# davidbau/rewriting

Measured on AMD Instinct MI355X. Metric: images/sec StyleGANv2-1024 fwd, higher is better.
Workload: dtype f32 (conv operands split into exact f16 pairs from 32x32 up, f32 accumulate); 1 GPU; stylegan2-1024 generator forward (FFHQ-1024 architecture); batch_per_gpu=64, mconv=seq, weights=synthetic seed 0, parallelism=seeds partitioned per rank, no collective, matrix_mode=split, direct_sums=auto

## Files before the change

rewriting_amd/csrc/rw_dconv.hip:

```cpp
#include "rw_common.h"

struct DconvProblem {
  const float* x; const unsigned char* wp; float* y;
  const float* style; const float* demod; const float* noise; const float* noise_w; const float* bias; int act;
  const float* post;
  const float* rgb_weight; const float* rgb_style; const float* rgb_bias; const float* rgb_skip; float* rgb_out;
  float rgb_scale;
  int batch, in_ch, out_ch, h, w;
  int tiles_x, tiles_y, o_tiles;
  int strided;
  float w_scale;
  float u_inv;
  const float* x_amax; float* y_amax;
};

#ifndef DC_ABL
#define DC_ABL 0
#endif
#define DC_PW 34
#ifndef DC_PROF
#define DC_PROF 0
#endif
#if DC_PROF
__device__ unsigned long long dc_prof[32];
extern "C" int rw_dconv_prof(unsigned long long* out) {
  return (int)hipMemcpyFromSymbol(out, HIP_SYMBOL(dc_prof), sizeof(unsigned long long) * 32);
}
#define DC_T() ((unsigned long long)clock64())
#endif

#ifndef DC_PRODUCTS
#define DC_PRODUCTS 3
#endif

__device__ __forceinline__ float dc_row_sum(float v) {
  v += __builtin_bit_cast(float, __builtin_amdgcn_update_dpp(0, __builtin_bit_cast(int, v), 0xB1, 0xf, 0xf, false));
  v += __builtin_bit_cast(float, __builtin_amdgcn_update_dpp(0, __builtin_bit_cast(int, v), 0x4E, 0xf, 0xf, false));
  v += __builtin_bit_cast(float, __builtin_amdgcn_update_dpp(0, __builtin_bit_cast(int, v), 0x141, 0xf, 0xf, false));
  v += __builtin_bit_cast(float, __builtin_amdgcn_update_dpp(0, __builtin_bit_cast(int, v), 0x140, 0xf, 0xf, false));
  return v;
}

template <int MODE, int WM>
__device__ __forceinline__ void dconv_body(const DconvProblem& p) {
  constexpr bool UP = MODE == 1, RGB = MODE == 2, RGBP = MODE == 3;
  static_assert(!RGB || WM == 1, "ToRGB: one wave holds all out-channels of its pixels");
  static_assert(!UP || WM == 2, "UP: the wave pairs are the two row phases");
  constexpr int WN = 4 / WM, TR = 4 * WN, PR = TR + 2;
  constexpr int NPIX = PR * DC_PW;
  constexpr int SI = (NPIX + 63) / 64;
  constexpr int BUFB = NPIX * 64;
  constexpr int VCH = 32 * WM;
  __shared__ __attribute__((aligned(16))) unsigned char Ls[2 * BUFB];
  __shared__ __attribute__((aligned(16))) float St[512];
  __shared__ float Ct[2][VCH];
  __shared__ float Cr[3][(RGB || RGBP) ? 32 * WM : 1];
  __shared__ float Red[4];

  const int tid = threadIdx.x, lane = tid & 63;
  const int wave = __builtin_amdgcn_readfirstlane(tid >> 6);
  const int wm = wave / WN, wn = wave % WN;
  const int lk = lane >> 4, lt = lane & 15;

  const int local = rw_xcd_remap(blockIdx.x, gridDim.x);
  const int ot = local % p.o_tiles;
  int pg = local / p.o_tiles;
  const int tx = pg % p.tiles_x; pg /= p.tiles_x;
  const int ty = pg % p.tiles_y;
  const int ib = pg / p.tiles_y;
  const int y0 = ty * TR, x0 = tx * 32;
  const int64_t hw = (int64_t)p.h * p.w;
  const int NC = p.in_ch >> 4, T = 9 * NC;
  const int real_ch = UP ? p.out_ch >> 2 : p.out_ch;

  float in_scale, out_scale;
  {
    float smax = p.style ? 0.f : 1.f;
    if (p.style)
      for (int i = tid; i < p.in_ch; i += 256) smax = fmaxf(smax, fabsf(p.style[(int64_t)ib * p.in_ch + i]));
    smax = rw_wave_max(smax);
    if (lane == 0) Red[wave] = smax;
    __syncthreads();
    smax = fmaxf(fmaxf(Red[0], Red[1]), fmaxf(Red[2], Red[3]));
    const float am = rw_bound_load(p.x_amax) * smax;
    int e = (int)((__float_as_uint(am) >> 23) & 0xff) - 126;
    e = e < -100 ? -100 : (e > 100 ? 100 : e);
    in_scale = __uint_as_float((unsigned)(127 + 14 - e) << 23);
    out_scale = __uint_as_float((unsigned)(127 + e - 14) << 23) * p.u_inv;
  }
  const float gain = p.act ? 1.4142135623730951f : 1.f, slope = p.act ? 0.2f : 1.f;
  for (int i = tid; i < p.in_ch; i += 256) St[i] = (p.style ? p.style[(int64_t)ib * p.in_ch + i] : 1.0f) * in_scale;
  if (tid < VCH) {
    const int o = UP ? 16 * ot + (tid & 15) : ot * VCH + tid;
    Ct[0][tid] = (p.demod ? p.demod[(int64_t)ib * real_ch + o] * p.w_scale : p.w_scale) * out_scale * gain;
    Ct[1][tid] = p.act ? p.bias[o] * gain : 0.f;
    if (RGB || RGBP) {
      const float sr = p.rgb_scale * p.rgb_style[(int64_t)ib * p.out_ch + o];
#pragma unroll
      for (int cc = 0; cc < 3; ++cc) Cr[cc][tid] = sr * p.rgb_weight[cc * p.out_ch + o];
    }
  }
  const float noise_wg = p.noise ? p.noise_w[0] * gain : 0.f;
  __syncthreads();

  const __amdgpu_buffer_rsrc_t xsrc = __builtin_amdgcn_make_buffer_rsrc(
      const_cast<float*>(p.x + (int64_t)ib * p.in_ch * hw), 0, (int)((int64_t)p.in_ch * hw * 4), 0x00020000);
  const int hw4 = (int)hw * 4;
  int xoff[SI], loff[SI];
#pragma unroll
  for (int s = 0; s < SI; ++s) {
    const int pi = 64 * s + lane;
    const int r = pi / DC_PW, cc = pi - r * DC_PW;
    const int iy = y0 - 1 + r, ix = x0 - 1 + cc;
    const bool ok = pi < NPIX && iy >= 0 && iy < p.h && ix >= 0 && ix < p.w;
    xoff[s] = ok ? (iy * p.w + ix) * 4 : 0x7fffffff;
    loff[s] = pi < NPIX ? pi * 64 + ((wave ^ rw_swz(cc)) << 4) : -1;
  }
  constexpr int SH = (SI + 1) / 2;
  float raw[SH][4];
  auto stage_load = [&](int c, auto half_tag) __attribute__((always_inline)) {
    constexpr int S0 = decltype(half_tag)::value ? SH : 0, S1 = decltype(half_tag)::value ? SI : SH;
    const int s0 = (16 * c + 4 * wave) * hw4;
#pragma unroll
    for (int s = S0; s < S1; ++s)
#pragma unroll
      for (int k = 0; k < 4; ++k)
        raw[s - S0][k] = (DC_ABL & 1) ? 1.f : __uint_as_float(__builtin_amdgcn_raw_buffer_load_b32(xsrc, xoff[s], s0 + k * hw4, 0));
  };
  auto stage_store = [&](int c, int buf, auto half_tag) __attribute__((always_inline)) {
    constexpr int S0 = decltype(half_tag)::value ? SH : 0, S1 = decltype(half_tag)::value ? SI : SH;
    const rw_f32x4 sv = *reinterpret_cast<const rw_f32x4*>(&St[16 * c + 4 * wave]);
    unsigned char* dst = Ls + buf * BUFB;
#pragma unroll
    for (int s = S0; s < S1; ++s) {
      const float (&rw)[4] = raw[s - S0];
      const float v0 = rw[0] * sv[0], v1 = rw[1] * sv[1], v2 = rw[2] * sv[2], v3 = rw[3] * sv[3];
      const rw_f16x2 h01 = __builtin_convertvector(rw_f32x2{v0, v1}, rw_f16x2);
      const rw_f16x2 h23 = __builtin_convertvector(rw_f32x2{v2, v3}, rw_f16x2);
      float r0, r1, r2, r3;
      asm("v_fma_mix_f32 %0, -%1, 1.0, %2 op_sel_hi:[1,0,0]" : "=v"(r0) : "v"(h01), "v"(v0));
      asm("v_fma_mix_f32 %0, -%1, 1.0, %2 op_sel:[1,0,0] op_sel_hi:[1,0,0]" : "=v"(r1) : "v"(h01), "v"(v1));
      asm("v_fma_mix_f32 %0, -%1, 1.0, %2 op_sel_hi:[1,0,0]" : "=v"(r2) : "v"(h23), "v"(v2));
      asm("v_fma_mix_f32 %0, -%1, 1.0, %2 op_sel:[1,0,0] op_sel_hi:[1,0,0]" : "=v"(r3) : "v"(h23), "v"(v3));
      const rw_f16x2 l01 = __builtin_convertvector(rw_f32x2{r0, r1}, rw_f16x2);
      const rw_f16x2 l23 = __builtin_convertvector(rw_f32x2{r2, r3}, rw_f16x2);
      const rw_f16x8 word = {h01[0], h01[1], h23[0], h23[1], l01[0], l01[1], l23[0], l23[1]};
      if (loff[s] >= 0) *reinterpret_cast<rw_f16x8*>(dst + loff[s]) = word;
    }
  };

  const int vb0 = ot * (2 * WM) + 2 * wm;
  const unsigned char* wbase = p.wp + (int64_t)vb0 * T * 1024 + lane * 8;
  rw_f16x8 W[3][2][2];
  rw_f32x2 Wc[3][2][2];
  auto wload = [&](int ky, int t) __attribute__((always_inline)) {
#pragma unroll
    for (int ob = 0; ob < 2; ++ob)
#pragma unroll
      for (int part = 0; part < 2; ++part) {
        if (DC_ABL & 4) Wc[ky][ob][part] = rw_f32x2{1.f, 1.f};
        else Wc[ky][ob][part] = *reinterpret_cast<const rw_f32x2*>(wbase + ((int64_t)ob * T + t) * 1024 + part * 512);
      }
  };
  auto wexpand = [&](int ky) __attribute__((always_inline)) {
#pragma unroll
    for (int ob = 0; ob < 2; ++ob) {
      W[ky][ob][0] = rw_expand(Wc[ky][ob][0]);
      if (DC_PRODUCTS == 4 || ky == 2) W[ky][ob][1] = rw_expand(Wc[ky][ob][1]);
      else if (ky == 1) W[0][ob][1] = rw_pair(Wc[0][ob][1], Wc[1][ob][1]);
    }
  };

  rw_f32x4 acc[2][8];
#pragma unroll
  for (int ob = 0; ob < 2; ++ob)
#pragma unroll
    for (int pb = 0; pb < 8; ++pb) acc[ob][pb] = rw_f32x4{0.f, 0.f, 0.f, 0.f};

  unsigned bbase[3];
#pragma unroll
  for (int kx = 0; kx < 3; ++kx) {
    const int cc = lt + kx;
    bbase[kx] = (unsigned)((4 * wn * DC_PW + cc) * 64 + ((lk ^ rw_swz(cc)) << 4));
  }
  auto bread = [&](const unsigned char* lb, int kx, int idx) __attribute__((always_inline)) {
    return *reinterpret_cast<const rw_f16x8*>(lb + bbase[kx] + ((idx >> 1) * DC_PW + 16 * (idx & 1)) * 64);
  };

  auto chunk = [&](int c, auto last_tag) __attribute__((always_inline)) {
    constexpr bool LAST = decltype(last_tag)::value != 0;
    const int buf = c & 1;
    const unsigned char* lb = Ls + buf * BUFB;
    if (!LAST) stage_load(c + 1, rw_int<0>());
    rw_f16x8 bcur = bread(lb, 0, 0);
    rw_f16x8 bprev[2] = {bcur, bcur};
#pragma unroll
    for (int kx = 0; kx < 3; ++kx) {
      const bool more = !LAST || kx < 2;
      const int tn = kx < 2 ? 9 * c + kx + 1 : 9 * (c + 1);
#pragma unroll
      for (int idx = 0; idx < 12; ++idx) {
        const int r = idx >> 1, half = idx & 1;
        if (half == 0 && r < 3) wexpand(r);
        rw_f16x8 bnext = bcur;
        if (idx + 1 < 12) bnext = bread(lb, kx, idx + 1);
        else if (kx < 2) bnext = bread(lb, kx + 1, 0);
#pragma unroll
        for (int ky = 0; ky < 3; ++ky) {
          const int pr = r - ky;
          if (pr < 0 || pr > 3) continue;
          const int pb = 2 * pr + half;
          if (DC_ABL & 2) { asm volatile("" :: "v"(bcur), "v"(W[ky][0][0]), "v"(W[ky][0][1]), "v"(W[ky][1][0]), "v"(W[ky][1][1])); continue; }
          acc[0][pb] = __builtin_amdgcn_mfma_f32_16x16x32_f16(bcur, W[ky][0][0], acc[0][pb], 0, 0, 0);
          acc[1][pb] = __builtin_amdgcn_mfma_f32_16x16x32_f16(bcur, W[ky][1][0], acc[1][pb], 0, 0, 0);
          if (DC_PRODUCTS == 4 || ky == 2) {
            acc[0][pb] = __builtin_amdgcn_mfma_f32_16x16x32_f16(bcur, W[ky][0][1], acc[0][pb], 0, 0, 0);
            acc[1][pb] = __builtin_amdgcn_mfma_f32_16x16x32_f16(bcur, W[ky][1][1], acc[1][pb], 0, 0, 0);
          }
        }
        if (DC_PRODUCTS == 3 && r >= 1 && r <= 4 && !(DC_ABL & 2)) {
          const int pb = 2 * (r - 1) + half;
          const rw_f16x8 hh = rw_pair(bprev[half], bcur);
          acc[0][pb] = __builtin_amdgcn_mfma_f32_16x16x32_f16(hh, W[0][0][1], acc[0][pb], 0, 0, 0);
          acc[1][pb] = __builtin_amdgcn_mfma_f32_16x16x32_f16(hh, W[0][1][1], acc[1][pb], 0, 0, 0);
        }
        bprev[half] = bcur;
        __builtin_amdgcn_sched_barrier(0);
        if (more && half == 1 && r >= 3) wload(r - 3, tn + 3 * (r - 3));
        bcur = bnext;
      }
      if (!LAST && kx == 0) {
        stage_store(c + 1, buf ^ 1, rw_int<0>());
        stage_load(c + 1, rw_int<1>());
      }
      __builtin_amdgcn_sched_barrier(0);
    }
    if (!LAST) {
      stage_store(c + 1, buf ^ 1, rw_int<1>());
      __syncthreads();
    }
  };

  wload(0, 0);
  wload(1, 3);
  wload(2, 6);
  stage_load(0, rw_int<0>());
  stage_store(0, 0, rw_int<0>());
  stage_load(0, rw_int<1>());
  stage_store(0, 0, rw_int<1>());
  __syncthreads();

  for (int c = 0; c + 1 < NC; ++c) chunk(c, rw_int<0>());
  chunk(NC - 1, rw_int<1>());
  if (DC_ABL & 8) { if (acc[0][0][0] != 12345.f) return; }

  float ymax = 0.f;
  if (MODE == 0 || RGBP) {
    const int oc = 16 * (2 * wm) + lt;
    const float sc[2] = {Ct[0][oc], Ct[0][oc + 16]}, bs[2] = {Ct[1][oc], Ct[1][oc + 16]};
    float* yb = p.y + ((int64_t)ib * p.out_ch + ot * VCH + oc) * hw;
    float cr[2][3] = {{0.f, 0.f, 0.f}, {0.f, 0.f, 0.f}};
    float* rb = nullptr;
    if (RGBP) {
#pragma unroll
      for (int ob = 0; ob < 2; ++ob)
#pragma unroll
        for (int cc = 0; cc < 3; ++cc) cr[ob][cc] = Cr[cc][oc + 16 * ob];
      rb = p.rgb_out + (((int64_t)(ot * WM + wm) * p.batch + ib) * 3 + (lt < 3 ? lt : 0)) * hw;
    }
#pragma unroll
    for (int pb = 0; pb < 8; ++pb) {
      const int64_t pix = (int64_t)(y0 + 4 * wn + (pb >> 1)) * p.w + x0 + 16 * (pb & 1) + 4 * lk;
      rw_f32x4 nz = {0.f, 0.f, 0.f, 0.f};
      if (p.noise) nz = *reinterpret_cast<const rw_f32x4*>(p.noise + (int64_t)ib * hw + pix) * noise_wg;
      rw_f32x4 v[2];
#pragma unroll
      for (int ob = 0; ob < 2; ++ob) {
#pragma unroll
        for (int j = 0; j < 4; ++j) {
          const float u = acc[ob][pb][j] * sc[ob] + nz[j] + bs[ob];
          v[ob][j] = fmaxf(u, u * slope);
          ymax = fmaxf(ymax, fabsf(v[ob][j]));
        }
        *reinterpret_cast<rw_f32x4*>(yb + (int64_t)(16 * ob) * hw + pix) = v[ob];
      }
      if (RGBP) {
        rw_f32x4 sum[3];
#pragma unroll
        for (int j = 0; j < 4; ++j)
#pragma unroll
          for (int cc = 0; cc < 3; ++cc) sum[cc][j] = dc_row_sum(v[0][j] * cr[0][cc] + v[1][j] * cr[1][cc]);
        if (lt < 3) *reinterpret_cast<rw_f32x4*>(rb + pix) = lt == 0 ? sum[0] : (lt == 1 ? sum[1] : sum[2]);
      }
    }
  } else if (UP) {
    const float sc = Ct[0][lt], bs = Ct[1][lt];
    const int ch = 16 * ot + lt;
    const float post = p.post ? p.post[(int64_t)ib * real_ch + ch] : 1.f;
    const int W2 = 2 * p.w;
    const int64_t hw2 = 4 * hw;
    float* yb = p.y + ((int64_t)ib * real_ch + ch) * hw2;
#pragma unroll
    for (int pb = 0; pb < 8; ++pb) {
      const int64_t pix = (int64_t)(2 * (y0 + 4 * wn + (pb >> 1)) + wm) * W2 + 2 * (x0 + 16 * (pb & 1) + 4 * lk);
      rw_f32x4 n0 = {0.f, 0.f, 0.f, 0.f}, n1 = n0;
      if (p.noise) {
        const float* np = p.noise + (int64_t)ib * hw2 + pix;
        n0 = *reinterpret_cast<const rw_f32x4*>(np) * noise_wg;
        n1 = *reinterpret_cast<const rw_f32x4*>(np + 4) * noise_wg;
      }
      rw_f32x4 q0 = {acc[0][pb][0], acc[1][pb][0], acc[0][pb][1], acc[1][pb][1]};
      rw_f32x4 q1 = {acc[0][pb][2], acc[1][pb][2], acc[0][pb][3], acc[1][pb][3]};
#pragma unroll
      for (int k = 0; k < 4; ++k) {
        const float u0 = q0[k] * sc + n0[k] + bs, u1 = q1[k] * sc + n1[k] + bs;
        q0[k] = fmaxf(u0, u0 * slope) * post; q1[k] = fmaxf(u1, u1 * slope) * post;
        ymax = fmaxf(ymax, fmaxf(fabsf(q0[k]), fabsf(q1[k])));
      }
      *reinterpret_cast<rw_f32x4*>(yb + pix) = q0;
      *reinterpret_cast<rw_f32x4*>(yb + pix + 4) = q1;
    }
  } else {
    const float sc[2] = {Ct[0][lt], Ct[0][lt + 16]}, bs[2] = {Ct[1][lt], Ct[1][lt + 16]};
    float cr[2][3];
#pragma unroll
    for (int ob = 0; ob < 2; ++ob)
#pragma unroll
      for (int cc = 0; cc < 3; ++cc) cr[ob][cc] = Cr[cc][lt + 16 * ob];
#pragma unroll
    for (int pb = 0; pb < 8; ++pb) {
      const int64_t pix = (int64_t)(y0 + 4 * wn + (pb >> 1)) * p.w + x0 + 16 * (pb & 1) + 4 * lk;
      rw_f32x4 nz = {0.f, 0.f, 0.f, 0.f};
      if (p.noise) nz = *reinterpret_cast<const rw_f32x4*>(p.noise + (int64_t)ib * hw + pix) * noise_wg;
      rw_f32x4 sum[3];
#pragma unroll
      for (int j = 0; j < 4; ++j) {
        float u0 = acc[0][pb][j] * sc[0] + nz[j] + bs[0], u1 = acc[1][pb][j] * sc[1] + nz[j] + bs[1];
        u0 = fmaxf(u0, u0 * slope); u1 = fmaxf(u1, u1 * slope);
#pragma unroll
        for (int cc = 0; cc < 3; ++cc) sum[cc][j] = dc_row_sum(u0 * cr[0][cc] + u1 * cr[1][cc]);
      }
      if (lt < 3) {
        const rw_f32x4 mine = lt == 0 ? sum[0] : (lt == 1 ? sum[1] : sum[2]);
        const int64_t off = ((int64_t)ib * 3 + lt) * hw + pix;
        rw_f32x4 o4 = mine + (p.rgb_bias ? p.rgb_bias[lt] : 0.f);
        if (p.rgb_skip) o4 += *reinterpret_cast<const rw_f32x4*>(p.rgb_skip + off);
        *reinterpret_cast<rw_f32x4*>(p.rgb_out + off) = o4;
      }
    }
  }
  if (!RGB && p.y_amax) rw_bound_store_wave(p.y_amax, rw_wave_max(ymax));
}

template <int MODE, int WM, int MW, int NL, int WC>
__device__ __forceinline__ void dconv_ws_body(const DconvProblem& p) {
  constexpr bool UP = MODE == 1, RGB = MODE == 2, RGBP = MODE == 3, PLAIN = MODE == 0 || MODE == 3;
  static_assert(!RGB || WM == 1, "ToRGB: one wave holds all out-channels of its pixels");
  static_assert(!UP || WM == 2, "UP: the wave pairs are the two row phases");
  constexpr int WN = MW / WM, WR = WN / WC, TR = 4 * WR, PR = TR + 2, TC = 32 * WC, PW = TC + 2;
  static_assert(WR * WC == WN && WR >= 1, "strips tile the workgroup's pixels");
  constexpr int QW = 4 / NL, NLL = 64 * NL;
  constexpr int NPIX = PR * PW, BUFB = NPIX * 64;
  constexpr int IPR = TC / 4 + 2, NITEM = PR * IPR, SI = (NITEM + 63) / 64;
  constexpr int VCH = 32 * WM;
  constexpr int WBUF = 2 * WM * 9 * 1024;
  __shared__ __attribute__((aligned(16))) unsigned char Ls[2 * BUFB];
  __shared__ __attribute__((aligned(16))) unsigned char Wl[2 * WBUF];
  __shared__ float Ct[2][2][VCH];
  __shared__ float Cr[2][3][VCH];
  __shared__ float Po[2][16];

  const int tid = threadIdx.x, lane = tid & 63;
  const int wave = __builtin_amdgcn_readfirstlane(tid >> 6);
  const int64_t hw = (int64_t)p.h * p.w;
  const int NC = p.in_ch >> 4, T = 9 * NC;
  const int real_ch = UP ? p.out_ch >> 2 : p.out_ch;
  const float gain = p.act ? 1.4142135623730951f : 1.f, slope = p.act ? 0.2f : 1.f;

  const int64_t total = (int64_t)p.batch * p.tiles_y * p.tiles_x * p.o_tiles;
  const int per = (int)((total + gridDim.x - 1) / gridDim.x);
  const int bx = p.strided ? rw_xcd_remap(blockIdx.x, gridDim.x) : blockIdx.x;
  const int t0 = p.strided ? 0 : bx * per;
  const int t1 = p.strided ? (int)((total - bx + gridDim.x - 1) / gridDim.x)
                           : (int)((int64_t)t0 + per < total ? t0 + per : total);
  if (t0 >= t1) {
    if (!RGB && p.y_amax) rw_bound_store_wave(p.y_amax, 0.f);
    return;
  }
  const int N = (t1 - t0) * NC;
  const int t_mul = p.strided ? gridDim.x : 1, t_add = p.strided ? bx : 0;
  auto decode = [&](int pos, int& ot, int& tx, int& ty, int& ib) __attribute__((always_inline)) {
    const int tile = pos * t_mul + t_add;
    ot = tile % p.o_tiles;
    int pg = tile / p.o_tiles;
    tx = pg % p.tiles_x; pg /= p.tiles_x;
    ty = pg % p.tiles_y;
    ib = pg / p.tiles_y;
  };
  auto lds_barrier = [&]() __attribute__((always_inline)) {
    asm volatile("" ::: "memory");
    __builtin_amdgcn_s_waitcnt(0xC07F);
    __builtin_amdgcn_s_barrier();
    asm volatile("" ::: "memory");
  };

  if (wave >= MW) {
    const int g2 = QW * (wave - MW), lid = (wave - MW) * 64 + lane;
    const float xam = rw_bound_load(p.x_amax);
    const int hw4 = (int)hw * 4;
    int loff[SI];
#pragma unroll
    for (int s = 0; s < SI; ++s) {
      const int it = 64 * s + lane;
      const int r = it / IPR, j = it - r * IPR;
      loff[s] = it < NITEM ? (r * PW + 4 * j - 3) * 64 : -1000000;
    }
    int l_tile = t0, l_c = 0, l_ib = -1, l_ot = 0, l_y0 = 0, l_x0 = 0;
    float in_scale = 1.f, out_scale = 1.f;
    int xoff[SI];
    __amdgpu_buffer_rsrc_t xsrc = __builtin_amdgcn_make_buffer_rsrc(const_cast<float*>(p.x), 0, 0, 0x00020000);
    rw_f32x4 raw[QW][SI][4];
    float psv[QW][4];
    float a_demod = 1.f, a_bias = 0.f, a_rgb = 0.f, a_post = 1.f, a_oscale = 1.f, a_iscale = 1.f;
    float a_crw[3] = {0.f, 0.f, 0.f};
    bool a_first = false;
    int a_par = 0;
    float crw[3] = {0.f, 0.f, 0.f};
    if (RGB && lid < 32) {
#pragma unroll
      for (int cc = 0; cc < 3; ++cc) crw[cc] = p.rgb_weight[cc * p.out_ch + lid] * p.rgb_scale;
    }

    float sv[QW][4];
    int l_s0 = 0;
    const unsigned char* l_wsrc = p.wp;
    auto setup = [&]() __attribute__((always_inline)) {
      if (l_tile >= t1) { l_tile = t1 - 1; l_c = NC - 1; }
      a_first = l_c == 0;
      if (l_c == 0) {
        int tx, ty, ib;
        decode(l_tile, l_ot, tx, ty, ib);
        l_y0 = ty * TR; l_x0 = tx * TC;
        if (ib != l_ib) {
          l_ib = ib;
          float smax = 0.f;
          for (int i = lane; i < p.in_ch; i += 64) smax = fmaxf(smax, fabsf(p.style[(int64_t)ib * p.in_ch + i]));
          smax = rw_wave_max(smax);
          const float am = xam * smax;
          int e = (int)((__float_as_uint(am) >> 23) & 0xff) - 126;
          e = e < -100 ? -100 : (e > 100 ? 100 : e);
          in_scale = __uint_as_float((unsigned)(127 + 14 - e) << 23);
          out_scale = __uint_as_float((unsigned)(127 + e - 14) << 23) * p.u_inv;
          xsrc = __builtin_amdgcn_make_buffer_rsrc(const_cast<float*>(p.x + (int64_t)ib * p.in_ch * hw), 0,
                                                   (int)((int64_t)p.in_ch * hw * 4), 0x00020000);
        }
#pragma unroll
        for (int s = 0; s < SI; ++s) {
          const int it = 64 * s + lane;
          const int r = it / IPR, j = it - r * IPR;
          const int iy = l_y0 - 1 + r, ix = l_x0 - 4 + 4 * j;
          const bool ok = it < NITEM && iy >= 0 && iy < p.h && ix >= 0 && ix < p.w;
          xoff[s] = ok ? (iy * p.w + ix) * 4 : 0x7ffffff0;
        }
        a_par = (l_tile - t0) & 1;
        a_oscale = out_scale;
        if (lid < VCH) {
          const int o = UP ? 16 * l_ot + (lid & 15) : l_ot * VCH + lid;
          a_demod = p.demod ? p.demod[(int64_t)l_ib * real_ch + o] : 1.f;
          a_bias = p.act ? p.bias[o] : 0.f;
          if (RGB || RGBP) a_rgb = p.rgb_style[(int64_t)l_ib * p.out_ch + o];
          if (RGBP) {
#pragma unroll
            for (int cc = 0; cc < 3; ++cc) a_crw[cc] = p.rgb_weight[cc * p.out_ch + o] * p.rgb_scale;
          }
          if (UP && lid < 16 && p.post) a_post = p.post[(int64_t)l_ib * real_ch + o];
        }
      }
#pragma unroll
      for (int q = 0; q < QW; ++q)
#pragma unroll
        for (int k = 0; k < 4; ++k) psv[q][k] = p.style[(int64_t)l_ib * p.in_ch + 16 * l_c + 4 * (g2 + q) + k];
      a_iscale = in_scale;
      l_s0 = (16 * l_c + 4 * g2) * hw4;
      l_wsrc = p.wp + ((int64_t)(l_ot * (2 * WM) + (wave - MW)) * T + 9 * l_c) * 1024;
      if (++l_c == NC) { l_c = 0; ++l_tile; }
    };
    static_assert(NL == 2 * WM && SI == 3, "wave j stages weight block j, three tap pieces per pixel piece");
    rw_f32x4 wraw[SI][3];
    auto request_s = [&](int s) __attribute__((always_inline)) {
#pragma unroll
      for (int q = 0; q < QW; ++q)
#pragma unroll
        for (int k = 0; k < 4; ++k) {
          if (DC_ABL & 1) raw[q][s][k] = rw_f32x4{1.f, 1.f, 1.f, 1.f};
          else raw[q][s][k] = __builtin_bit_cast(rw_f32x4, __builtin_amdgcn_raw_buffer_load_b128(xsrc, xoff[s], l_s0 + (4 * q + k) * hw4, 0));
        }
#pragma unroll
      for (int k = 0; k < 3; ++k) {
        if (DC_ABL & 4) wraw[s][k] = rw_f32x4{1.f, 1.f, 1.f, 1.f};
        else wraw[s][k] = *reinterpret_cast<const rw_f32x4*>(l_wsrc + (3 * s + k) * 1024 + lane * 16);
      }
    };
    auto tables = [&]() __attribute__((always_inline)) {
#pragma unroll
      for (int q = 0; q < QW; ++q)
#pragma unroll
        for (int k = 0; k < 4; ++k) sv[q][k] = psv[q][k] * a_iscale;
      if (a_first) {
        if (lid < VCH) {
          Ct[a_par][0][lid] = a_demod * p.w_scale * a_oscale * gain;
          Ct[a_par][1][lid] = a_bias * gain;
          if (RGB || RGBP) {
#pragma unroll
            for (int cc = 0; cc < 3; ++cc) Cr[a_par][cc][lid] = a_rgb * (RGBP ? a_crw[cc] : crw[cc]);
          }
          if (UP && lid < 16) Po[a_par][lid] = a_post;
        }
      }
    };
    auto deliver_s = [&](int buf, int s) __attribute__((always_inline)) {
      unsigned char* dst = Ls + buf * BUFB;
      unsigned char* wdst = Wl + buf * WBUF + (wave - MW) * 9216 + lane * 16;
#pragma unroll
      for (int k = 0; k < 3; ++k) *reinterpret_cast<rw_f32x4*>(wdst + (3 * s + k) * 1024) = wraw[s][k];
      const int it = 64 * s + lane;
      const int j = it % IPR;
#pragma unroll
      for (int q = 0; q < QW; ++q)
#pragma unroll
        for (int e = 0; e < 4; ++e) {
          const float v0 = raw[q][s][0][e] * sv[q][0], v1 = raw[q][s][1][e] * sv[q][1], v2 = raw[q][s][2][e] * sv[q][2],
                      v3 = raw[q][s][3][e] * sv[q][3];
          const rw_f16x2 h01 = __builtin_convertvector(rw_f32x2{v0, v1}, rw_f16x2);
          const rw_f16x2 h23 = __builtin_convertvector(rw_f32x2{v2, v3}, rw_f16x2);
          float r0, r1, r2, r3;
          asm("v_fma_mix_f32 %0, -%1, 1.0, %2 op_sel_hi:[1,0,0]" : "=v"(r0) : "v"(h01), "v"(v0));
          asm("v_fma_mix_f32 %0, -%1, 1.0, %2 op_sel:[1,0,0] op_sel_hi:[1,0,0]" : "=v"(r1) : "v"(h01), "v"(v1));
          asm("v_fma_mix_f32 %0, -%1, 1.0, %2 op_sel_hi:[1,0,0]" : "=v"(r2) : "v"(h23), "v"(v2));
          asm("v_fma_mix_f32 %0, -%1, 1.0, %2 op_sel:[1,0,0] op_sel_hi:[1,0,0]" : "=v"(r3) : "v"(h23), "v"(v3));
          const rw_f16x2 l01 = __builtin_convertvector(rw_f32x2{r0, r1}, rw_f16x2);
          const rw_f16x2 l23 = __builtin_convertvector(rw_f32x2{r2, r3}, rw_f16x2);
          const rw_f16x8 word = {h01[0], h01[1], h23[0], h23[1], l01[0], l01[1], l23[0], l23[1]};
          const int cc = 4 * j - 3 + e;
          if (it < NITEM && cc >= 0 && cc < PW)
            *reinterpret_cast<rw_f16x8*>(dst + loff[s] + e * 64 + (((g2 + q) ^ rw_swz(cc)) << 4)) = word;
        }
    };

    setup();
#pragma unroll
    for (int s = 0; s < SI; ++s) request_s(s);
    tables();
    __builtin_amdgcn_sched_barrier(0);
    setup();
#pragma unroll
    for (int s = 0; s < SI; ++s) { deliver_s(0, s); __builtin_amdgcn_sched_barrier(0); request_s(s); __builtin_amdgcn_sched_barrier(0); }
    lds_barrier();
#if DC_PROF
    unsigned long long pt_del = 0, pt_req = 0, pt_bar = 0, pt_all = DC_T();
#endif
    for (int n = 0; n < N; ++n) {
#if DC_PROF
      const unsigned long long ta = DC_T();
#endif
      tables();
      __builtin_amdgcn_sched_barrier(0);
      setup();
#if DC_PROF
      const unsigned long long tb = DC_T();
#endif
#pragma unroll
      for (int s = 0; s < SI; ++s) { deliver_s((n + 1) & 1, s); __builtin_amdgcn_sched_barrier(0); request_s(s); __builtin_amdgcn_sched_barrier(0); }
#if DC_PROF
      const unsigned long long tc = DC_T();
#endif
      lds_barrier();
#if DC_PROF
      const unsigned long long td = DC_T();
      pt_del += tb - ta; pt_req += tc - tb; pt_bar += td - tc;
#endif
    }
#if DC_PROF
    if (wave == MW && lane == 0 && (blockIdx.x == 0 || blockIdx.x == 100)) {
      unsigned long long* o = dc_prof + (blockIdx.x == 0 ? 0 : 16);
      o[8] = DC_T() - pt_all; o[9] = pt_del; o[10] = pt_req; o[11] = pt_bar; o[12] = N;
    }
#endif
    if (!RGB && p.y_amax) rw_bound_store_wave(p.y_amax, 0.f);
    return;
  }

  const int wm = wave / WN, wn = wave % WN, wr = wn / WC, wc = wn % WC;
  const int lk = lane >> 4, lt = lane & 15;
  unsigned bbase[3];
#pragma unroll
  for (int kx = 0; kx < 3; ++kx) {
    const int cc = lt + kx;
    bbase[kx] = (unsigned)((4 * wr * PW + 32 * wc + cc) * 64 + ((lk ^ rw_swz(cc)) << 4));
  }
  auto bread = [&](const unsigned char* lb, int kx, int idx) __attribute__((always_inline)) {
    return *reinterpret_cast<const rw_f16x8*>(lb + bbase[kx] + ((idx >> 1) * PW + 16 * (idx & 1)) * 64);
  };
  rw_f16x8 W[3][2];
  rw_f32x2 Wc[3][2];
  auto wread = [&](const unsigned char* wb, int kx, int part) __attribute__((always_inline)) {
#pragma unroll
    for (int ky = 0; ky < 3; ++ky)
#pragma unroll
      for (int ob = 0; ob < 2; ++ob) {
        if (DC_ABL & 4) Wc[ky][ob] = rw_f32x2{1.f, 1.f};
        else Wc[ky][ob] = *reinterpret_cast<const rw_f32x2*>(wb + ((2 * wm + ob) * 9 + 3 * ky + kx) * 1024 + part * 512 + lane * 8);
      }
  };
  const float noise_wg = p.noise ? p.noise_w[0] * gain : 0.f;
  rw_f32x4 nzp[PLAIN ? 8 : 1];
  rw_f32x4 acc[2][8];
#pragma unroll
  for (int ob = 0; ob < 2; ++ob)
#pragma unroll
    for (int pb = 0; pb < 8; ++pb) acc[ob][pb] = rw_f32x4{0.f, 0.f, 0.f, 0.f};
  float ymax = 0.f;
  float rgb_b[3] = {0.f, 0.f, 0.f};
  if (RGB && p.rgb_bias) { rgb_b[0] = p.rgb_bias[0]; rgb_b[1] = p.rgb_bias[1]; rgb_b[2] = p.rgb_bias[2]; }

  int tile = t0, c = 0;
  int ot, tx, ty, ib;
  decode(tile, ot, tx, ty, ib);
  lds_barrier();

#if DC_PROF
  unsigned long long pt_mm = 0, pt_bar = 0, pt_epi = 0, pt_all = DC_T();
#endif
  for (int n = 0; n < N; ++n) {
#if DC_PROF
    const unsigned long long ta = DC_T();
#endif
    const unsigned char* lb = Ls + (n & 1) * BUFB;
    const unsigned char* wb = Wl + (n & 1) * WBUF;
    if (PLAIN && c == NC - 1 && p.noise) {
      const float* np = p.noise + (int64_t)ib * hw + (int64_t)(ty * TR + 4 * wr) * p.w + tx * TC + 32 * wc + 4 * lk;
#pragma unroll
      for (int pb = 0; pb < 8; ++pb) nzp[pb] = *reinterpret_cast<const rw_f32x4*>(np + (int64_t)(pb >> 1) * p.w + 16 * (pb & 1));
    }
    rw_f16x8 bq[3];
    wread(wb, 0, 0);
    bq[0] = bread(lb, 0, 0);
    bq[1] = bread(lb, 0, 1);
    rw_f16x8 bprev[2] = {bq[0], bq[1]};
#pragma unroll
    for (int hs = 0; hs < 6; ++hs) {
      const int kx = hs >> 1, part = hs & 1;
#pragma unroll
      for (int ob = 0; ob < 2; ++ob) {
        if (DC_PRODUCTS == 4 || part == 0) {
#pragma unroll
          for (int ky = 0; ky < 3; ++ky) W[ky][ob] = rw_expand(Wc[ky][ob]);
        } else {
          W[0][ob] = rw_pair(Wc[0][ob], Wc[1][ob]);
          W[2][ob] = rw_expand(Wc[2][ob]);
        }
      }
      __builtin_amdgcn_sched_barrier(0);
      if (hs + 1 < 6) wread(wb, (hs + 1) >> 1, (hs + 1) & 1);
      __builtin_amdgcn_sched_barrier(0);
#pragma unroll
      for (int idx = 0; idx < 12; ++idx) {
        const int r = idx >> 1, half = idx & 1;
        const rw_f16x8 b = bq[idx % 3];
        if (idx + 2 < 12) bq[(idx + 2) % 3] = bread(lb, kx, idx + 2);
        else if (hs < 5) bq[(idx + 2) % 3] = bread(lb, (hs + 1) >> 1, idx + 2 - 12);
        if (DC_PRODUCTS == 4 || part == 0) {
#pragma unroll
          for (int ky = 0; ky < 3; ++ky) {
            const int pr = r - ky;
            if (pr < 0 || pr > 3) continue;
            const int pb = 2 * pr + half;
            if (DC_ABL & 2) { asm volatile("" :: "v"(b), "v"(W[ky][0]), "v"(W[ky][1])); continue; }
            acc[0][pb] = __builtin_amdgcn_mfma_f32_16x16x32_f16(b, W[ky][0], acc[0][pb], 0, 0, 0);
            acc[1][pb] = __builtin_amdgcn_mfma_f32_16x16x32_f16(b, W[ky][1], acc[1][pb], 0, 0, 0);
          }
        } else if (DC_ABL & 2) {
          asm volatile("" :: "v"(b), "v"(W[0][0]), "v"(W[0][1]), "v"(W[2][0]), "v"(W[2][1]));
        } else {
          if (r >= 1 && r <= 4) {
            const int pb = 2 * (r - 1) + half;
            const rw_f16x8 hh = rw_pair(bprev[half], b);
            acc[0][pb] = __builtin_amdgcn_mfma_f32_16x16x32_f16(hh, W[0][0], acc[0][pb], 0, 0, 0);
            acc[1][pb] = __builtin_amdgcn_mfma_f32_16x16x32_f16(hh, W[0][1], acc[1][pb], 0, 0, 0);
          }
          if (r >= 2) {
            const int pb = 2 * (r - 2) + half;
            acc[0][pb] = __builtin_amdgcn_mfma_f32_16x16x32_f16(b, W[2][0], acc[0][pb], 0, 0, 0);
            acc[1][pb] = __builtin_amdgcn_mfma_f32_16x16x32_f16(b, W[2][1], acc[1][pb], 0, 0, 0);
          }
          bprev[half] = b;
        }
        __builtin_amdgcn_sched_barrier(0);
      }
    }
#if DC_PROF
    const unsigned long long tb = DC_T();
#endif
    lds_barrier();
#if DC_PROF
    const unsigned long long tc = DC_T();
    pt_mm += tb - ta; pt_bar += tc - tb;
    if (c + 1 == NC) pt_epi -= tc;
#endif
    if (++c < NC) continue;
    c = 0;
    const int par = (tile - t0) & 1;
    const int y0 = ty * TR, x0 = tx * TC;
    if (!(DC_ABL & 8)) {
      if (PLAIN) {
        const int oc = 16 * (2 * wm) + lt;
        const float sc[2] = {Ct[par][0][oc], Ct[par][0][oc + 16]}, bs[2] = {Ct[par][1][oc], Ct[par][1][oc + 16]};
        float* yb = p.y + ((int64_t)ib * p.out_ch + ot * VCH + oc) * hw;
        float cr[2][3] = {{0.f, 0.f, 0.f}, {0.f, 0.f, 0.f}};
        float* rb = nullptr;
        if (RGBP) {
#pragma unroll
          for (int ob = 0; ob < 2; ++ob)
#pragma unroll
            for (int cc = 0; cc < 3; ++cc) cr[ob][cc] = Cr[par][cc][oc + 16 * ob];
          rb = p.rgb_out + (((int64_t)(ot * WM + wm) * p.batch + ib) * 3 + (lt < 3 ? lt : 0)) * hw;
        }
#pragma unroll
        for (int pb = 0; pb < 8; ++pb) {
          const int64_t pix = (int64_t)(y0 + 4 * wr + (pb >> 1)) * p.w + x0 + 32 * wc + 16 * (pb & 1) + 4 * lk;
          rw_f32x4 nz = {0.f, 0.f, 0.f, 0.f};
          if (p.noise) nz = nzp[pb] * noise_wg;
          rw_f32x4 v[2];
#pragma unroll
          for (int ob = 0; ob < 2; ++ob) {
#pragma unroll
            for (int j = 0; j < 4; ++j) {
              const float u = acc[ob][pb][j] * sc[ob] + nz[j] + bs[ob];
              v[ob][j] = fmaxf(u, u * slope);
              ymax = fmaxf(ymax, fabsf(v[ob][j]));
            }
            if (!(DC_ABL & 16)) *reinterpret_cast<rw_f32x4*>(yb + (int64_t)(16 * ob) * hw + pix) = v[ob];
          }
          if (RGBP) {
            rw_f32x4 sum[3];
#pragma unroll
            for (int j = 0; j < 4; ++j)
#pragma unroll
              for (int cc = 0; cc < 3; ++cc) sum[cc][j] = dc_row_sum(v[0][j] * cr[0][cc] + v[1][j] * cr[1][cc]);
            if (lt < 3 && !(DC_ABL & 16)) *reinterpret_cast<rw_f32x4*>(rb + pix) = lt == 0 ? sum[0] : (lt == 1 ? sum[1] : sum[2]);
          }
        }
      } else if (UP) {
        const float sc = Ct[par][0][lt], bs = Ct[par][1][lt];
        const int ch = 16 * ot + lt;
        const float post = Po[par][lt];
        const int W2 = 2 * p.w;
        float* yb = p.y + ((int64_t)ib * real_ch + ch) * (4 * hw);
#pragma unroll
        for (int pb = 0; pb < 8; ++pb) {
          const int orow = 2 * (4 * wr + (pb >> 1)) + wm, ocol = 2 * (32 * wc + 16 * (pb & 1) + 4 * lk);
          const int64_t pix = (int64_t)(2 * y0 + orow) * W2 + 2 * x0 + ocol;
          rw_f32x4 n0 = {0.f, 0.f, 0.f, 0.f}, n1 = n0;
          if (p.noise) {
            const float* np = p.noise + (int64_t)ib * (4 * hw) + pix;
            n0 = *reinterpret_cast<const rw_f32x4*>(np) * noise_wg;
            n1 = *reinterpret_cast<const rw_f32x4*>(np + 4) * noise_wg;
          }
          rw_f32x4 q0 = {acc[0][pb][0], acc[1][pb][0], acc[0][pb][1], acc[1][pb][1]};
          rw_f32x4 q1 = {acc[0][pb][2], acc[1][pb][2], acc[0][pb][3], acc[1][pb][3]};
#pragma unroll
          for (int k = 0; k < 4; ++k) {
            const float u0 = q0[k] * sc + n0[k] + bs, u1 = q1[k] * sc + n1[k] + bs;
            q0[k] = fmaxf(u0, u0 * slope) * post; q1[k] = fmaxf(u1, u1 * slope) * post;
            ymax = fmaxf(ymax, fmaxf(fabsf(q0[k]), fabsf(q1[k])));
          }
          if (!(DC_ABL & 16)) {
            *reinterpret_cast<rw_f32x4*>(yb + pix) = q0;
            *reinterpret_cast<rw_f32x4*>(yb + pix + 4) = q1;
          }
        }
      } else {
        const float sc[2] = {Ct[par][0][lt], Ct[par][0][lt + 16]}, bs[2] = {Ct[par][1][lt], Ct[par][1][lt + 16]};
        float cr[2][3];
#pragma unroll
        for (int ob = 0; ob < 2; ++ob)
#pragma unroll
          for (int cc = 0; cc < 3; ++cc) cr[ob][cc] = Cr[par][cc][lt + 16 * ob];
#pragma unroll
        for (int pb = 0; pb < 8; ++pb) {
          const int64_t pix = (int64_t)(y0 + 4 * wr + (pb >> 1)) * p.w + x0 + 32 * wc + 16 * (pb & 1) + 4 * lk;
          rw_f32x4 nz = {0.f, 0.f, 0.f, 0.f};
          if (p.noise) nz = *reinterpret_cast<const rw_f32x4*>(p.noise + (int64_t)ib * hw + pix) * noise_wg;
          rw_f32x4 sum[3];
#pragma unroll
          for (int j = 0; j < 4; ++j) {
            float u0 = acc[0][pb][j] * sc[0] + nz[j] + bs[0], u1 = acc[1][pb][j] * sc[1] + nz[j] + bs[1];
            u0 = fmaxf(u0, u0 * slope); u1 = fmaxf(u1, u1 * slope);
#pragma unroll
            for (int cc = 0; cc < 3; ++cc) sum[cc][j] = dc_row_sum(u0 * cr[0][cc] + u1 * cr[1][cc]);
          }
          if (lt < 3) {
            const rw_f32x4 mine = lt == 0 ? sum[0] : (lt == 1 ? sum[1] : sum[2]);
            const int64_t off = ((int64_t)ib * 3 + lt) * hw + pix;
            rw_f32x4 o4 = mine + (lt == 0 ? rgb_b[0] : (lt == 1 ? rgb_b[1] : rgb_b[2]));
            if (p.rgb_skip) o4 += *reinterpret_cast<const rw_f32x4*>(p.rgb_skip + off);
            *reinterpret_cast<rw_f32x4*>(p.rgb_out + off) = o4;
          }
        }
      }
    }
#pragma unroll
    for (int ob = 0; ob < 2; ++ob)
#pragma unroll
      for (int pb = 0; pb < 8; ++pb) acc[ob][pb] = rw_f32x4{0.f, 0.f, 0.f, 0.f};
    if (++tile < t1) decode(tile, ot, tx, ty, ib);
#if DC_PROF
    pt_epi += DC_T();
#endif
  }
#if DC_PROF
  if (wave == 0 && lane == 0 && (blockIdx.x == 0 || blockIdx.x == 100)) {
    unsigned long long* o = dc_prof + (blockIdx.x == 0 ? 0 : 16);
    o[0] = DC_T() - pt_all; o[1] = pt_mm; o[2] = pt_bar; o[3] = pt_epi; o[4] = N;
  }
#endif
  if (!RGB && p.y_amax) rw_bound_store_wave(p.y_amax, rw_wave_max(ymax));
}

__global__ void __launch_bounds__(768, 3) dconv_ws_w2_kernel(const DconvProblem p) { dconv_ws_body<0, 2, 8, 4, 2>(p); }
__global__ void __launch_bounds__(768, 3) dconv_ws_up_kernel(const DconvProblem p) { dconv_ws_body<1, 2, 8, 4, 2>(p); }
__global__ void __launch_bounds__(768, 3) dconv_ws_w2_rgbp_kernel(const DconvProblem p) { dconv_ws_body<3, 2, 8, 4, 2>(p); }
__global__ void __launch_bounds__(384, 2) dconv_ws_rgb_kernel(const DconvProblem p) { dconv_ws_body<2, 1, 4, 2, 2>(p); }

__global__ void __launch_bounds__(256, 2) dconv_w1_kernel(const DconvProblem p) { dconv_body<0, 1>(p); }
__global__ void __launch_bounds__(256, 2) dconv_w2_kernel(const DconvProblem p) { dconv_body<0, 2>(p); }
__global__ void __launch_bounds__(256, 2) dconv_w4_kernel(const DconvProblem p) { dconv_body<0, 4>(p); }
__global__ void __launch_bounds__(256, 2) dconv_up_kernel(const DconvProblem p) { dconv_body<1, 2>(p); }
__global__ void __launch_bounds__(256, 2) dconv_rgb_kernel(const DconvProblem p) { dconv_body<2, 1>(p); }
__global__ void __launch_bounds__(256, 2) dconv_w1_rgbp_kernel(const DconvProblem p) { dconv_body<3, 1>(p); }
__global__ void __launch_bounds__(256, 2) dconv_w2_rgbp_kernel(const DconvProblem p) { dconv_body<3, 2>(p); }
__global__ void __launch_bounds__(256, 2) dconv_w4_rgbp_kernel(const DconvProblem p) { dconv_body<3, 4>(p); }

template <int PASS, bool UP>
__global__ void __launch_bounds__(256) pack_dconv_kernel(const float* __restrict__ w, const float* __restrict__ k4,
                                                         unsigned char* __restrict__ wp, float* __restrict__ trailer,
                                                         int vch, int in_ch, float su, float* __restrict__ bound) {
  const int64_t total = (int64_t)vch * in_ch;
  const int NC = in_ch >> 4, T = 9 * NC;
  float m = 0.f;
  for (int64_t idx = (int64_t)blockIdx.x * blockDim.x + threadIdx.x; idx < total; idx += (int64_t)gridDim.x * blockDim.x) {
    const int i = (int)(idx % in_ch), v = (int)(idx / in_ch);
    const int vb = v >> 4, n = v & 15;
    float h[9];
    if (UP) {
      const int ot = vb >> 2, py = (vb >> 1) & 1, px = vb & 1;
      const float* g = w + ((int64_t)(16 * ot + n) * in_ch + i) * 9;
#pragma unroll
      for (int a = 0; a < 3; ++a)
#pragma unroll
        for (int b = 0; b < 3; ++b) {
          const int ty = 2 - 2 * a + py, tx = 2 - 2 * b + px;
          float sum = 0.f;
#pragma unroll
          for (int c = 0; c < 4; ++c)
#pragma unroll
            for (int d = 0; d < 4; ++d) {
              const int ky = ty - 1 + c, kx = tx - 1 + d;
              if (ky >= 0 && ky < 3 && kx >= 0 && kx < 3) sum += k4[(3 - c) * 4 + (3 - d)] * g[3 * ky + kx];
            }
          h[3 * a + b] = sum;
        }
    } else {
      const float* g = w + ((int64_t)v * in_ch + i) * 9;
#pragma unroll
      for (int t = 0; t < 9; ++t) h[t] = g[t];
    }
    if (PASS == 1) {
#pragma unroll
      for (int t = 0; t < 9; ++t) m = fmaxf(m, fabsf(h[t]));
      continue;
    }
    const int c = i >> 4, g4 = (i & 15) >> 2, k = i & 3, lane = 16 * g4 + n;
    _Float16* dst = reinterpret_cast<_Float16*>(wp + ((int64_t)vb * T + 9 * c) * 1024) + lane * 4 + k;
#pragma unroll
    for (int t = 0; t < 9; ++t) {
      const float u = h[t] * su;
      const _Float16 hi = (_Float16)u;
      const _Float16 lo = (_Float16)(u - (float)hi);
      _Float16* d = dst + t * 512;
      d[0] = hi;
      d[256] = lo;
    }
  }
  __shared__ float red[4];
  if (PASS == 1) rw_bound_store_block_256(bound, m, red);
  if (PASS == 2 && blockIdx.x == 0 && threadIdx.x < 4)
    trailer[threadIdx.x] = threadIdx.x == 0 ? 1.f / su : (threadIdx.x == 1 ? su : 0.f);
}

static bool dconv_specialised(int in_ch, const rw_conv_epilogue* ep) {
  return in_ch >= 32 && ep && ep->style && !rw_env_is("RW_DCONV_V", '1');
}
static unsigned dconv_ws_grid(int64_t tiles, int per_cu = 1) {
  int64_t g = rw_env_int("RW_DCONV_GRID", rw_cu_count() * per_cu);
  if (g < 1) g = 1;
  return (unsigned)(tiles < g ? tiles : g);
}

static bool dconv_shape_ok(int out_ch, int in_ch, int h, int w) {
  return out_ch > 0 && out_ch % 32 == 0 && in_ch >= 16 && in_ch % 16 == 0 && in_ch <= 512 && w % 32 == 0 && h % 16 == 0;
}

extern "C" int rw_dconv3x3_supported(int out_ch, int in_ch, int h, int w) { return dconv_shape_ok(out_ch, in_ch, h, w) ? 1 : 0; }

extern "C" long long rw_packed_dconv_weight_elems(int out_ch, int in_ch) {
  if (out_ch <= 0 || in_ch <= 0 || out_ch % 16 || in_ch % 16) return -1;
  return 9LL * out_ch * in_ch + 4;
}

template <bool UP>
static int dconv_absmax(const float* w, const float* k4, int vch, int in_ch, float* bound, rw_stream_t stream) {
  const int64_t total = (int64_t)vch * in_ch;
  const int grid = rw_stream_grid(total, 256);
  hipLaunchKernelGGL((pack_dconv_kernel<1, UP>), dim3(grid), dim3(256), 0, rw_s(stream), w, k4, (unsigned char*)nullptr,
                     (float*)nullptr, vch, in_ch, 1.f, bound);
  return rw_finish_bound(bound, grid, stream);
}

template <bool UP>
static int dconv_pack(const float* w, const float* k4, float* wp, int vch, int in_ch, float u_scale, rw_stream_t stream) {
  const int64_t total = (int64_t)vch * in_ch;
  float* trailer = wp + 9 * total;
  unsigned char* bytes = reinterpret_cast<unsigned char*>(wp);
  hipLaunchKernelGGL((pack_dconv_kernel<2, UP>), dim3(rw_stream_grid(total, 256)), dim3(256), 0, rw_s(stream), w, k4, bytes,
                     trailer, vch, in_ch, u_scale, (float*)nullptr);
  return RW_LAUNCH_RESULT();
}

extern "C" int rw_dconv_weight_absmax_f32(const float* w, int out_ch, int in_ch, float* bound, rw_stream_t stream) {
  RW_CHECK_ARG(w && bound && out_ch > 0 && in_ch > 0);
  if (out_ch % 16 || in_ch % 16) return RW_ERR_UNSUPPORTED;
  return dconv_absmax<false>(w, nullptr, out_ch, in_ch, bound, stream);
}

extern "C" int rw_pack_dconv_weight_f32(const float* w, float* wp, int out_ch, int in_ch, float u_scale, rw_stream_t stream) {
  RW_CHECK_ARG(w && wp && out_ch > 0 && in_ch > 0 && u_scale > 0.f);
  if (out_ch % 16 || in_ch % 16) return RW_ERR_UNSUPPORTED;
  return dconv_pack<false>(w, nullptr, wp, out_ch, in_ch, u_scale, stream);
}

static void dconv_fill(DconvProblem& p, const float* x, const float* wp, int batch, int in_ch, int vch, int h, int w,
                       float w_scale, const rw_conv_epilogue* ep, float u_inv, const float* x_amax, float* y_amax) {
  p.x = x; p.wp = reinterpret_cast<const unsigned char*>(wp);
  p.u_inv = u_inv;
  rw_fill_epilogue(p, ep);
  p.batch = batch; p.in_ch = in_ch; p.out_ch = vch; p.h = h; p.w = w; p.w_scale = w_scale;
  p.x_amax = x_amax; p.y_amax = y_amax;
  p.tiles_x = w / 32;
  p.strided = rw_env_int("RW_DCONV_ORDER", 1);
}

static int dconv3x3_launch(const float* x, const float* wp, float* y, int batch, int in_ch, int out_ch, int h, int w,
                           float w_scale, const rw_conv_epilogue* ep, const rw_rgb_epilogue* rgb, float u_inv,
                           const float* x_amax, float* y_amax, rw_stream_t stream) {
  if (!dconv_shape_ok(out_ch, in_ch, h, w)) return RW_ERR_UNSUPPORTED;
  if ((int64_t)in_ch * h * w * 4 > 0x7fffffffLL) return RW_ERR_UNSUPPORTED;
  DconvProblem p = {};
  dconv_fill(p, x, wp, batch, in_ch, out_ch, h, w, w_scale, ep, u_inv, x_amax, y_amax);
  p.y = y;
  if (rgb) { p.rgb_weight = rgb->weight; p.rgb_style = rgb->style; p.rgb_out = rgb->out; p.rgb_scale = rgb->scale; }
  const int64_t cap = rw_bound_slot_capacity((int64_t)batch * out_ch * h * w);
  int wm = out_ch % 128 == 0 ? 4 : (out_ch % 64 == 0 ? 2 : 1);
  const int force = rw_env_int("RW_DCONV_WM", 0);
  if ((force == 1 || force == 2 || force == 4) && out_ch % (32 * force) == 0) wm = force;
  p.o_tiles = out_ch / (32 * wm);
  p.tiles_y = h / (16 / wm);
  const int64_t work = (int64_t)batch * p.tiles_y * p.tiles_x * p.o_tiles;
  if (work <= 0 || work > 0x7fffffff) return RW_ERR_UNSUPPORTED;
  if (dconv_specialised(in_ch, ep) && out_ch % 64 == 0 && h % 8 == 0 && w % 64 == 0) {
    p.o_tiles = out_ch / 64; p.tiles_y = h / 8; p.tiles_x = w / 64;
    const unsigned grid = dconv_ws_grid((int64_t)batch * p.tiles_y * p.tiles_x * p.o_tiles);
    if (y_amax && 12LL * grid > cap) return RW_ERR_UNSUPPORTED;
    void (*const ws_kernel)(DconvProblem) = rgb ? dconv_ws_w2_rgbp_kernel : dconv_ws_w2_kernel;
    hipLaunchKernelGGL(ws_kernel, dim3(grid), dim3(768), 0, rw_s(stream), p);
    return rw_finish_bound(y_amax, 12LL * grid, stream);
  }
  if (y_amax && 4 * work > cap) return RW_ERR_UNSUPPORTED;
  void (*const kernel)(DconvProblem) = wm == 4 ? (rgb ? dconv_w4_rgbp_kernel : dconv_w4_kernel)
                                     : wm == 2 ? (rgb ? dconv_w2_rgbp_kernel : dconv_w2_kernel)
                                               : (rgb ? dconv_w1_rgbp_kernel : dconv_w1_kernel);
  hipLaunchKernelGGL(kernel, dim3((unsigned)work), dim3(256), 0, rw_s(stream), p);
  return rw_finish_bound(y_amax, 4 * work, stream);
}

extern "C" int rw_dconv3x3_f32(const float* x, const float* wp, float* y, int batch, int in_ch, int out_ch, int h, int w,
                               float w_scale, const rw_conv_epilogue* ep, float u_inv, const float* x_amax, float* y_amax,
                               rw_stream_t stream) {
  RW_CHECK_ARG(x && wp && y && x_amax && u_inv > 0.f && batch > 0 && in_ch > 0 && out_ch > 0 && h > 0 && w > 0);
  RW_CHECK_ARG(rw_epilogue_ok(ep));
  return dconv3x3_launch(x, wp, y, batch, in_ch, out_ch, h, w, w_scale, ep, nullptr, u_inv, x_amax, y_amax, stream);
}

extern "C" int rw_dconv3x3_rgb_partials(int out_ch) { return out_ch > 0 && out_ch % 32 == 0 ? out_ch / 32 : -1; }
extern "C" int rw_dconv3x3_rgb_partial_f32(const float* x, const float* wp, float* y, int batch, int in_ch, int out_ch, int h,
                                           int w, float w_scale, const rw_conv_epilogue* ep, const rw_rgb_epilogue* rgb,
                                           float u_inv, const float* x_amax, float* y_amax, rw_stream_t stream) {
  RW_CHECK_ARG(x && wp && y && x_amax && u_inv > 0.f && batch > 0 && in_ch > 0 && out_ch > 0 && h > 0 && w > 0);
  RW_CHECK_ARG(rw_rgb_ok(rgb));
  RW_CHECK_ARG(rw_epilogue_ok(ep));
  return dconv3x3_launch(x, wp, y, batch, in_ch, out_ch, h, w, w_scale, ep, rgb, u_inv, x_amax, y_amax, stream);
}

static bool dconv_up_shape_ok(int out_ch, int in_ch, int h, int w) {
  return out_ch > 0 && out_ch % 16 == 0 && in_ch >= 16 && in_ch % 16 == 0 && in_ch <= 512 && w % 32 == 0 && h % 8 == 0;
}
extern "C" int rw_dconv_transpose_blur_supported(int out_ch, int in_ch, int h, int w) {
// ... 73 lines not shown
```

Measured before the change: 1591 images/sec.

## Pair tap-2 low-order products across kx=0,1 to cut split-precision MFMAs

Extends the split-f16 product-pairing trick to the ky=2 taps. Previously only the ky=0/1 low parts shared an MFMA. Now the low-order weight halves for kx=0 and kx=1 of row ky=2 are packed into one K=32 operand. The matching activation halves are packed the same way, which removes one pair of MFMAs per pixel block in both the dconv body and the plain/RGBP kernel. The cost is extra half-width LDS reads, a few more registers to stage the kx=0 weights, and an opaque lane copy in the epilogue that is likely there to control register pressure.

```diff
diff --git a/rewriting_amd/csrc/rw_dconv.hip b/rewriting_amd/csrc/rw_dconv.hip
--- a/rewriting_amd/csrc/rw_dconv.hip
+++ b/rewriting_amd/csrc/rw_dconv.hip
@@ -32,6 +32,10 @@
 #ifndef DC_PRODUCTS
 #define DC_PRODUCTS 3
 #endif
+#ifndef DC_TAP2_PAIR
+#define DC_TAP2_PAIR 1
+#endif
+#define DC_T2P (DC_PRODUCTS == 3 && DC_TAP2_PAIR)
 
 __device__ __forceinline__ float dc_row_sum(float v) {
   v += __builtin_bit_cast(float, __builtin_amdgcn_update_dpp(0, __builtin_bit_cast(int, v), 0xB1, 0xf, 0xf, false));
@@ -153,6 +157,7 @@
   const unsigned char* wbase = p.wp + (int64_t)vb0 * T * 1024 + lane * 8;
   rw_f16x8 W[3][2][2];
   rw_f32x2 Wc[3][2][2];
+  rw_f32x2 Wk[2] = {};
   auto wload = [&](int ky, int t) __attribute__((always_inline)) {
 #pragma unroll
     for (int ob = 0; ob < 2; ++ob)
@@ -162,11 +167,13 @@
         else Wc[ky][ob][part] = *reinterpret_cast<const rw_f32x2*>(wbase + ((int64_t)ob * T + t) * 1024 + part * 512);
       }
   };
-  auto wexpand = [&](int ky) __attribute__((always_inline)) {
+  auto wexpand = [&](int ky, int kx) __attribute__((always_inline)) {
 #pragma unroll
     for (int ob = 0; ob < 2; ++ob) {
       W[ky][ob][0] = rw_expand(Wc[ky][ob][0]);
-      if (DC_PRODUCTS == 4 || ky == 2) W[ky][ob][1] = rw_expand(Wc[ky][ob][1]);
+      if (DC_T2P && ky == 2 && kx == 0) Wk[ob] = Wc[2][ob][1];
+      else if (DC_T2P && ky == 2 && kx == 1) W[2][ob][1] = rw_pair(Wk[ob], Wc[2][ob][1]);
+      else if (DC_PRODUCTS == 4 || ky == 2) W[ky][ob][1] = rw_expand(Wc[ky][ob][1]);
       else if (ky == 1) W[0][ob][1] = rw_pair(Wc[0][ob][1], Wc[1][ob][1]);
     }
   };
@@ -185,6 +192,9 @@
   }
   auto bread = [&](const unsigned char* lb, int kx, int idx) __attribute__((always_inline)) {
     return *reinterpret_cast<const rw_f16x8*>(lb + bbase[kx] + ((idx >> 1) * DC_PW + 16 * (idx & 1)) * 64);
+  };
+  auto bread_h = [&](const unsigned char* lb, int kx, int idx) __attribute__((always_inline)) {
+    return *reinterpret_cast<const rw_f32x2*>(lb + bbase[kx] + ((idx >> 1) * DC_PW + 16 * (idx & 1)) * 64);
   };
 
   auto chunk = [&](int c, auto last_tag) __attribute__((always_inline)) {
@@ -201,10 +211,12 @@
 #pragma unroll
       for (int idx = 0; idx < 12; ++idx) {
         const int r = idx >> 1, half = idx & 1;
-        if (half == 0 && r < 3) wexpand(r);
+        if (half == 0 && r < 3) wexpand(r, kx);
         rw_f16x8 bnext = bcur;
         if (idx + 1 < 12) bnext = bread(lb, kx, idx + 1);
         else if (kx < 2) bnext = bread(lb, kx + 1, 0);
+        rw_f32x2 bh0 = {};
+        if (DC_T2P && kx == 1 && r >= 2 && !(DC_ABL & 2)) bh0 = bread_h(lb, 0, idx);
 #pragma unroll
         for (int ky = 0; ky < 3; ++ky) {
           const int pr = r - ky;
@@ -213,10 +225,17 @@
           if (DC_ABL & 2) { asm volatile("" :: "v"(bcur), "v"(W[ky][0][0]), "v"(W[ky][0][1]), "v"(W[ky][1][0]), "v"(W[ky][1][1])); continue; }
           acc[0][pb] = __builtin_amdgcn_mfma_f32_16x16x32_f16(bcur, W[ky][0][0], acc[0][pb], 0, 0, 0);
           acc[1][pb] = __builtin_amdgcn_mfma_f32_16x16x32_f16(bcur, W[ky][1][0], acc[1][pb], 0, 0, 0);
+          if (DC_T2P && ky == 2 && kx < 2) continue;
           if (DC_PRODUCTS == 4 || ky == 2) {
             acc[0][pb] = __builtin_amdgcn_mfma_f32_16x16x32_f16(bcur, W[ky][0][1], acc[0][pb], 0, 0, 0);
             acc[1][pb] = __builtin_amdgcn_mfma_f32_16x16x32_f16(bcur, W[ky][1][1], acc[1][pb], 0, 0, 0);
           }
+        }
+        if (DC_T2P && kx == 1 && r >= 2 && !(DC_ABL & 2)) {
+          const int pb = 2 * (r - 2) + half;
+          const rw_f16x8 hh = rw_pair(rw_expand(bh0), bcur);
+          acc[0][pb] = __builtin_amdgcn_mfma_f32_16x16x32_f16(hh, W[2][0][1], acc[0][pb], 0, 0, 0);
+          acc[1][pb] = __builtin_amdgcn_mfma_f32_16x16x32_f16(hh, W[2][1][1], acc[1][pb], 0, 0, 0);
         }
         if (DC_PRODUCTS == 3 && r >= 1 && r <= 4 && !(DC_ABL & 2)) {
           const int pb = 2 * (r - 1) + half;
@@ -601,13 +620,22 @@
   auto bread = [&](const unsigned char* lb, int kx, int idx) __attribute__((always_inline)) {
     return *reinterpret_cast<const rw_f16x8*>(lb + bbase[kx] + ((idx >> 1) * PW + 16 * (idx & 1)) * 64);
   };
+  constexpr bool T2P1 = DC_T2P && !(DC_ABL & 2);
+  auto bread_hs = [&](const unsigned char* lb, int hs, int idx) __attribute__((always_inline)) {
+    const unsigned off = ((idx >> 1) * PW + 16 * (idx & 1)) * 64;
+    if (T2P1 && hs == 3)
+      return rw_pair(*reinterpret_cast<const rw_f32x2*>(lb + bbase[1] + off), *reinterpret_cast<const rw_f32x2*>(lb + bbase[0] + off));
+    return bread(lb, hs >> 1, idx);
+  };
   rw_f16x8 W[3][2];
   rw_f32x2 Wc[3][2];
+  rw_f32x2 Wk[2] = {};
   auto wread = [&](const unsigned char* wb, int kx, int part) __attribute__((always_inline)) {
 #pragma unroll
     for (int ky = 0; ky < 3; ++ky)
 #pragma unroll
       for (int ob = 0; ob < 2; ++ob) {
+        if (DC_T2P && part == 1 && ky == 2 && kx == 0) continue;
         if (DC_ABL & 4) Wc[ky][ob] = rw_f32x2{1.f, 1.f};
         else Wc[ky][ob] = *reinterpret_cast<const rw_f32x2*>(wb + ((2 * wm + ob) * 9 + 3 * ky + kx) * 1024 + part * 512 + lane * 8);
       }
@@ -657,7 +685,8 @@
           for (int ky = 0; ky < 3; ++ky) W[ky][ob] = rw_expand(Wc[ky][ob]);
         } else {
           W[0][ob] = rw_pair(Wc[0][ob], Wc[1][ob]);
-          W[2][ob] = rw_expand(Wc[2][ob]);
+          if (DC_T2P && kx == 1) W[2][ob] = rw_pair(Wc[2][ob], Wk[ob]);
+          else if (!(DC_T2P && kx == 0)) W[2][ob] = rw_expand(Wc[2][ob]);
         }
       }
       __builtin_amdgcn_sched_barrier(0);
@@ -667,8 +696,15 @@
       for (int idx = 0; idx < 12; ++idx) {
         const int r = idx >> 1, half = idx & 1;
         const rw_f16x8 b = bq[idx % 3];
-        if (idx + 2 < 12) bq[(idx + 2) % 3] = bread(lb, kx, idx + 2);
-        else if (hs < 5) bq[(idx + 2) % 3] = bread(lb, (hs + 1) >> 1, idx + 2 - 12);
+        if (idx + 2 < 12) bq[(idx + 2) % 3] = bread_hs(lb, hs, idx + 2);
+        else if (hs < 5) bq[(idx + 2) % 3] = bread_hs(lb, hs + 1, idx + 2 - 12);
+        if (T2P1 && hs == 2 && idx == 10) {
+#pragma unroll
+          for (int ob = 0; ob < 2; ++ob) {
+            if (DC_ABL & 4) Wk[ob] = rw_f32x2{1.f, 1.f};
+            else Wk[ob] = *reinterpret_cast<const rw_f32x2*>(wb + ((2 * wm + ob) * 9 + 6) * 1024 + 512 + lane * 8);
+          }
+        }
         if (DC_PRODUCTS == 4 || part == 0) {
 #pragma unroll
           for (int ky = 0; ky < 3; ++ky) {
@@ -680,7 +716,8 @@
             acc[1][pb] = __builtin_amdgcn_mfma_f32_16x16x32_f16(b, W[ky][1], acc[1][pb], 0, 0, 0);
           }
         } else if (DC_ABL & 2) {
-          asm volatile("" :: "v"(b), "v"(W[0][0]), "v"(W[0][1]), "v"(W[2][0]), "v"(W[2][1]));
+          if (DC_T2P && kx == 0) asm volatile("" :: "v"(b), "v"(W[0][0]), "v"(W[0][1]));
+          else asm volatile("" :: "v"(b), "v"(W[0][0]), "v"(W[0][1]), "v"(W[2][0]), "v"(W[2][1]));
         } else {
           if (r >= 1 && r <= 4) {
             const int pb = 2 * (r - 1) + half;
@@ -688,7 +725,7 @@
             acc[0][pb] = __builtin_amdgcn_mfma_f32_16x16x32_f16(hh, W[0][0], acc[0][pb], 0, 0, 0);
             acc[1][pb] = __builtin_amdgcn_mfma_f32_16x16x32_f16(hh, W[0][1], acc[1][pb], 0, 0, 0);
           }
-          if (r >= 2) {
+          if (r >= 2 && !(DC_T2P && kx == 0)) {
             const int pb = 2 * (r - 2) + half;
             acc[0][pb] = __builtin_amdgcn_mfma_f32_16x16x32_f16(b, W[2][0], acc[0][pb], 0, 0, 0);
             acc[1][pb] = __builtin_amdgcn_mfma_f32_16x16x32_f16(b, W[2][1], acc[1][pb], 0, 0, 0);
@@ -712,6 +749,9 @@
     const int par = (tile - t0) & 1;
     const int y0 = ty * TR, x0 = tx * TC;
     if (!(DC_ABL & 8)) {
+      int lane_e = lane;
+      asm volatile("" : "+v"(lane_e));
+      const int lk = lane_e >> 4, lt = lane_e & 15;
       if (PLAIN) {
         const int oc = 16 * (2 * wm) + lt;
         const float sc[2] = {Ct[par][0][oc], Ct[par][0][oc + 16]}, bs[2] = {Ct[par][1][oc], Ct[par][1][oc + 16]};
```

New measurement: 1625 images/sec, median of 6. +2.1%, better.
